# markosski/immutable3

Measured on AMD Instinct MI355X. Metric: scanned rows/sec + %HBM-roofline, 100M-row RangeFilter, 1/2/4/8 MI355X, higher is better.
Workload: dtype i32; 1 GPU; C2@100M: RangeFilter GT(2^28) AND LT(3*2^28) over one 100M-row DENSE_INT segment -> selection bitmap + selected-row count; block_rows=1024, segments_rotated_per_gpu=3, parallelism=1 GPU

## Files before the change

immutable3_amd/csrc/imm3_api.cpp:

```cpp
#include "../../include/imm3.h"
#include "../../include/imm3_diag.h"
#include "imm3_internal.h"
#include "../host/codec.hpp"

#include <algorithm>
#include <cmath>
#include <map>
#include <mutex>
#include <unordered_map>
#include <cstdio>
#include <cstring>
#include <functional>
#include <memory>
#include <string>
#include <vector>

#include "imm3_handles.h"
#include "imm3_distinct_plan.h"
#include "imm3_api_internal.h"

using namespace imm3;

static thread_local std::string g_err;

// ... 636 lines not shown
    const size_t bytes = (size_t)rows * 2 + kPad;
    void *p = nullptr, *pm = nullptr;
    if (rows < 1 || hipMalloc(&p, bytes) != hipSuccess || hipMalloc(&pm, 2 * sizeof(int32_t)) != hipSuccess) {
        (void)hipGetLastError();
        if (p) (void)hipFree(p);
        sc.hi16_state = -1;
        return IMM3_OK;
    }
    int32_t min_max[2] = {32767, -32768};
    hipError_t e = hipMemcpyAsync(pm, min_max, sizeof(min_max), hipMemcpyHostToDevice, ctx->stream);
    if (e == hipSuccess) e = hipMemsetAsync((uint8_t *)p + (size_t)rows * 2, 0, kPad, ctx->stream);
    if (e == hipSuccess) {
        LaunchTimer t(ctx, 5);
        launch_hi16_build((const int32_t *)sc.d_data, (int16_t *)p, rows, (int32_t *)pm, ctx->stream, t.start, t.stop);
        e = hipGetLastError();
    }
    if (e == hipSuccess) e = hipMemcpyAsync(min_max, pm, sizeof(min_max), hipMemcpyDeviceToHost, ctx->stream);
    if (e == hipSuccess) e = hipStreamSynchronize(ctx->stream);
    (void)hipFree(pm);
    if (e != hipSuccess) {
        (void)hipFree(p);
        HIPCHK(e);
    }
    if (!hi16_span_ok(min_max[0], min_max[1])) {
        (void)hipFree(p);
        sc.hi16_state = -1;
        return IMM3_OK;
    }
    sc.d_hi16 = (uint8_t *)p;
    sc.hi16_state = 1;
    seg->device_bytes += bytes;
    return IMM3_OK;
}

static int segment_await(imm3_ctx *ctx, const imm3_segment *seg) {
    if (seg->ready_pending.load(std::memory_order_acquire)) HIPCHK(hipStreamWaitEvent(ctx->stream, seg->ready, 0));
    return IMM3_OK;
}

static int segment_build(imm3_ctx *ctx, const imm3_column *cols, int32_t ncols, bool wrap, imm3_segment **out, bool async = false) {
    if (!out) return fail(IMM3_ERR_ARG, "null argument");
    *out = nullptr;
    CTX_LIVE(ctx);
    if (ncols <= 0 || !cols) return fail(IMM3_ERR_ARG, "a segment needs at least one column");
    HIPCHK(hipSetDevice(ctx->device));
    std::unique_ptr<imm3_segment, void (*)(imm3_segment *)> seg(new imm3_segment(), segment_free);
// ... 70 lines not shown
    }
    for (void *p : seg->registered) unpin_range(seg->ctx, p);
    seg->registered.clear();
    return IMM3_OK;
}

extern "C" int imm3_segment_destroy(imm3_segment *seg) {
    if (!seg) return IMM3_OK;
    if (seg->closed) return fail(IMM3_ERR_STATE, "segment destroyed twice");
    imm3_ctx *ctx = seg->ctx;
    ctx_retain(ctx);
    struct Unref { imm3_ctx *c; ~Unref() { ctx_release(c); } } unref{ctx};
    imm3::GateScope gate(&ctx->gate);
    if (!ctx->closed && ctx->capture) return fail(IMM3_ERR_STATE, "a graph capture is open on this context");
    seg->closed = true;
    if (!seg->ctx->closed) {
        (void)hipSetDevice(seg->ctx->device);
        if (seg->ready_pending.load()) (void)hipEventSynchronize(seg->ready);
        (void)hipStreamSynchronize(seg->ctx->stream);
    }
    for (void *p : seg->registered) unpin_range(seg->ctx, p);
    seg->registered.clear();
    segment_release(seg);
    return IMM3_OK;
}

extern "C" int imm3_segment_bytes(const imm3_segment *seg, uint64_t *device_bytes) {
    if (!seg || !device_bytes) return fail(IMM3_ERR_ARG, "null argument");
    *device_bytes = seg->device_bytes;
    return IMM3_OK;
}

static void table_release(const imm3_table *t);

static void query_free(imm3_query *q) {
    if (!q) return;
    imm3_ctx *ctx = q->ctx;
    if (!ctx) { delete q; return; }
    (void)hipSetDevice(ctx->device);
    if (ctx->aux && q->total_on_aux) (void)hipStreamSynchronize(ctx->aux);
    pool_release(ctx, q->d_bitmap);
    pool_release(ctx, q->d_tile_offsets);
    pool_release(ctx, q->d_chunk_sums);
    pool_release(ctx, q->d_block_partials);
    pool_release(ctx, q->d_limit_state);
    pool_release(ctx, q->d_total);
// ... 1072 lines not shown
            const size_t j = (size_t)(which - IMM3_PTR_ORDER_COLUMN);
            *ptr = j < q->d_order_proj.size() ? q->d_order_proj[j] : nullptr;
            return IMM3_OK;
        }
        if (which >= 16 && (size_t)(which - 16) < q->d_proj.size()) {
            *ptr = q->d_proj[(size_t)(which - 16)];
            return IMM3_OK;
        }
        return fail(IMM3_ERR_ARG, "unknown device pointer id");
    }
}

extern "C" int imm3_query_plan(const imm3_query *q, int64_t *out, int32_t n) {
    if (!q || !out) return fail(IMM3_ERR_ARG, "null argument");
    const int64_t v[15] = {q->single_pass ? 1 : 0, q->sp_P, q->sp_grid, q->sp_spans, q->d_stage_rec ? 1 : 0,
                           (q->single_pass || q->d_stage_rec) ? rec_layout(q->stage_kinds, -1).dwords : 0, q->run.ran_single_pass ? 1 : 0, (int64_t)q->run_syncs,
                           (int64_t)q->sp_abandoned_runs, (int64_t)q->sp_busy_runs, (int64_t)q->limit_gather_gave_up,
                           (int64_t)q->order_select_runs, (int64_t)q->order_full_runs, (int64_t)q->order_launches,
                           q->hi16_ran ? 1 : 0};
    for (int32_t i = 0; i < n && i < 15; ++i) out[i] = v[i];
    return IMM3_OK;
}

static int query_create_agg_impl(imm3_ctx *ctx, const imm3_segment *seg, const imm3_table *table,
                                 const int32_t *used_cols, int32_t n_used,
                                 const imm3_select *sels, int32_t n_sels,
                                 const int32_t *group_cols, int32_t n_group,
                                 const imm3_aggregate *aggs, int32_t n_aggs,
                                 int32_t table_block_size, imm3_query **out, bool wide_keys,
                                 const int32_t *prog = nullptr, int32_t n_prog = 0, bool tree = false) {
    if (!out) return fail(IMM3_ERR_ARG, "out is null");
    *out = nullptr;
    if (n_group < 0 || n_group > kMaxGroupCols || (n_group > 0 && !group_cols)) return fail(IMM3_ERR_ARG, "0..4 group columns are supported on the GPU path");
    if (n_aggs < 1 || n_aggs > kMaxAggs || !aggs) return fail(IMM3_ERR_ARG, "1..4 aggregates are supported on the GPU path");
    imm3_query *q = nullptr;
    std::vector<int32_t> row_cols(group_cols, group_cols + n_group);
    for (int32_t j = 0; j < n_aggs; ++j) row_cols.push_back(aggs[j].column);
    int rc = query_create_impl(ctx, seg, table, used_cols, n_used, sels, n_sels, nullptr, 0, 0, table_block_size, row_cols, &q, prog, n_prog, tree);
    if (rc) return rc;
    std::unique_ptr<imm3_query, void (*)(imm3_query *)> guard(q, query_free);
    int key_bytes = 0;
    for (int32_t g = 0; g < n_group; ++g) {
        if (group_cols[g] < 0 || group_cols[g] >= n_used) return fail(IMM3_ERR_ARG, "group column is not among the used columns");
        key_bytes += seg->cols[(size_t)q->used[(size_t)group_cols[g]]].width;
    }
    if (!wide_keys && key_bytes > 8) return fail(IMM3_ERR_ARG, "group key wider than 8 bytes is not supported on the GPU path");
// ... 540 lines not shown
```

immutable3_amd/csrc/imm3_handles.h:

```cpp
#pragma once

#include "../../include/imm3.h"
#include "imm3_internal.h"
#include "imm3_plan.h"
#include "imm3_sync.h"

#include <atomic>
#include <map>
#include <memory>
#include <mutex>
#include <string>
#include <unordered_map>
#include <vector>

namespace imm3 {
int fail(int code, const std::string &msg);
}
using imm3::fail;

#define HIPCHK(expr)                                                                              \
    do {                                                                                          \
        hipError_t _e = (expr);                                                                   \
        if (_e != hipSuccess)                                                                     \
            return fail(IMM3_ERR_DEVICE, std::string(#expr) + ": " + hipGetErrorString(_e));      \
// ... 112 lines not shown
static inline int32_t value_codec(int32_t c) {
    if (c == IMM3_PFOR_INT || c == IMM3_SNAPPY_INT) return IMM3_DENSE_INT;
    if (c == IMM3_SNAPPY_TINYINT) return IMM3_DENSE_TINYINT;
    if (c == IMM3_SNAPPY_STRING) return IMM3_DENSE_STRING;
    return c;
}

struct SegCol {
    int32_t codec = 0, width = 0;
    int32_t vcodec = 0;
    uint8_t *d_data = nullptr;
    bool owned = false;
    uint64_t bytes = 0;
    std::vector<int32_t> offsets;
    std::vector<int32_t> block_rows;
    int32_t in_cap = 0, out_cap = 0;
    int64_t rows = 0;
    bool tile_aligned = false;
    uint32_t *d_block_off = nullptr;
    uint32_t *d_row_base = nullptr;
    uint8_t *d_dense = nullptr;
    uint8_t *d_hi16 = nullptr;
    int32_t hi16_state = 0;
};

struct SegLayout {
    std::vector<int32_t> size;
    std::vector<int64_t> word_off;
    int64_t rows = 0, words = 0;
    bool ragged = false;
};

struct imm3_segment {
    std::atomic<int> refs{1};
    std::atomic<bool> closed{false};
    imm3_ctx *ctx = nullptr;
    std::vector<SegCol> cols;
    uint64_t device_bytes = 0;
    std::vector<void *> registered;
    hipEvent_t ready = nullptr;
    std::atomic<bool> ready_pending{false};
    std::mutex decode_mu;
    std::mutex layout_mu;
    std::map<int32_t, std::shared_ptr<const SegLayout>> layouts;
    std::map<std::pair<int32_t, int32_t>, bool> same_blocks;
    std::map<int32_t, void **> d_sample_ptrs;
// ... 185 lines not shown
```

immutable3_amd/csrc/imm3_internal.h:

```cpp
#pragma once

#include <hip/hip_runtime.h>
#include <stdint.h>
#include <algorithm>

#include "imm3_int_list_plan.h"
#include "imm3_hi16_plan.h"

#ifdef IMM3_ABLATE
#define IMM3_ABLATED(args, value) ((args).ablate == (value))
#define IMM3_ABLATE_BIT(args, bit) (((args).ablate & (bit)) != 0)
#else
#define IMM3_ABLATED(args, value) false
#define IMM3_ABLATE_BIT(args, bit) false
#endif

namespace imm3 {

constexpr int kTileRows = 1024;
constexpr int kTileWords = 16;
constexpr int kWavesPerBlock = 4;
constexpr int kBlockThreads = 256;
constexpr int kChunkTiles = 256;
constexpr int kSpanTiles = 16;
// ... 19 lines not shown
    int32_t list;
    int32_t list_empty;
    uint32_t list_mask, list_shift, list_max_probe;
};

enum TileKind : int32_t { TK_I32 = 0, TK_I8 = 1, TK_S2 = 2, TK_NONE = 3, TK_H16 = 4 };
constexpr int tile_kind_rank(int kind) { return kind == TK_H16 ? 3 : (kind == TK_NONE ? 4 : kind); }
constexpr int kMaxTileCols = 3;
constexpr int kDeferLines = 64;
constexpr int kMaxTileMatch = 8;
constexpr int kMaxArenaSlots = 256;

struct TileCol {
    const void *data;
    int32_t lo, hi;
    int32_t n_match;
    int32_t negated;
    uint32_t match[kMaxTileMatch];
};
IMM3_HOST_DEVICE inline const void *tile_col_full(const TileCol &c) { return (const void *)(uintptr_t)(((uint64_t)c.match[5] << 32) | (uint64_t)c.match[4]); }
inline void tile_col_set_full(TileCol &c, const void *full) {
    c.match[4] = (uint32_t)(uintptr_t)full;
    c.match[5] = (uint32_t)((uint64_t)(uintptr_t)full >> 32);
}

struct TileArgs {
    TileCol cols[kMaxTileCols];
    int32_t kinds[kMaxTileCols];
    int32_t and_existing;
    int32_t defer_lines;
    int32_t ablate;
    int64_t n_rows, n_words, n_tiles;
    uint64_t *bitmap;
    uint32_t *block_partials;
    unsigned long long *finish;
    void *stage_rec;
    uint32_t *tile_start;
    int64_t wave_cap;
    int32_t max_slots;
    int32_t chunked;
    unsigned long long *stamps;
    const uint32_t *tile_rows;
    const void *const *tile_ptrs[kMaxTileCols];
};

struct RecField {
// ... 89 lines not shown
};
void launch_emit(const EmitArgs &a, int n_gather, int grid_blocks, hipStream_t s, hipEvent_t ev0, hipEvent_t ev1);

constexpr int kProjectMinP = 1;
constexpr int kProjectMaxP = 64;
#ifndef IMM3_PROJECT_STREAMERS
#define IMM3_PROJECT_STREAMERS 8
#endif
#ifndef IMM3_PROJECT_RING_KB
#define IMM3_PROJECT_RING_KB 14
#endif
constexpr int kProjectStreamers = IMM3_PROJECT_STREAMERS;
constexpr int kProjectWriters = 4;
constexpr int kProjectRingBytes = IMM3_PROJECT_RING_KB * 1024;
constexpr int kFinishStatus = 2;
constexpr unsigned long long kStatusPfor = 1ULL, kStatusAbandoned = 2ULL, kStatusBusy = 4ULL;
constexpr int kStatusEpochShift = 8;
constexpr unsigned long long kStatusEpochMask = 0xFFFFFFULL;
constexpr int kFinishEpoch = 8;
constexpr int kFinishDense = 9;
constexpr int kFinishLimitRows = 11;
constexpr int kFinishLimitTiles = 12;
constexpr int kFinishLimitGaveUp = 13;
constexpr int kFinishLimitTicketLineWord = 8;
constexpr int kTableLimitMaxGrid = 512;
constexpr int kTableLimitClaimTiles = 32;
static_assert(kTableLimitClaimTiles % kSpanTiles == 0 && kTableLimitClaimTiles % kWavesPerBlock == 0, "the scanned prefix ends on a span boundary; a claim splits evenly over the waves");
constexpr int kDescValueBits = 36, kDescFlagShift = 36, kDescEpochShift = 38;
constexpr unsigned long long kDescValueMask = (1ULL << kDescValueBits) - 1;
constexpr unsigned long long kDescEpochMask = (1ULL << (64 - kDescEpochShift)) - 1;
constexpr uint32_t kProjectMaxPolls = 1u << 17;
struct ProjectTile {
    const void *p[kMaxTileCols];
    uint32_t rows;
    uint32_t pad;
};
struct ProjectArgs {
    TileCol cols[kMaxTileCols];
    int32_t kinds[kMaxTileCols];
    int32_t P;
    int64_t n_rows, n_tiles, n_spans;
    int64_t n_rounds;
    uint64_t *bitmap;
    unsigned long long *finish;
    unsigned long long *desc;
    unsigned long long *round_total;
// ... 304 lines not shown
    uint32_t slots, mask;
    const unsigned long long *recs;
    uint32_t n_recs;
    unsigned long long *out_recs;
    unsigned long long *out_n;
    uint32_t out_cap;
};
void launch_mergew_pack(const MergeWideArgs &a, hipStream_t s);
void launch_mergew_init(const MergeWideArgs &a, hipStream_t s);
void launch_mergew_insert(const MergeWideArgs &a, hipStream_t s);
void launch_mergew_collect(const MergeWideArgs &a, hipStream_t s);
void launch_group_collect(const AggArgs &a, hipStream_t s);
void launch_strmax_init(const AggArgs &a, hipStream_t s);
void launch_strmax_refine(const AggArgs &a, int j, int k, hipStream_t s, hipEvent_t ev0, hipEvent_t ev1);
void launch_strmax_collect(const AggArgs &a, int j, uint32_t n_groups, uint8_t *out, hipStream_t s);
void launch_distinct_mark(const AggArgs &a, int j, hipStream_t s, hipEvent_t ev0, hipEvent_t ev1);
void launch_group_keys(const AggArgs &a, uint32_t n_groups, int key_bytes, uint8_t *out, hipStream_t s);

constexpr int kSubTallies = 32;
constexpr int kFinishWords = 16 + kSubTallies * 16;
constexpr int kFinishLimitTicket = 16 + 16 * (kSubTallies - 1) + kFinishLimitTicketLineWord;
static_assert(kFinishLimitTicket < kFinishWords && kFinishLimitTicketLineWord > 0 && kFinishLimitTicketLineWord < 16, "the ticket word lies inside the finish block, beside the last sub-tally");
constexpr int kMaxFilterGrid = 4096;
int filter_grid(int64_t units, bool generic, bool any_i32, int grid_blocks, int narrow_row_bytes = 0);
struct PforArgs {
    const uint8_t *data;
    const uint32_t *block_off;
    const uint32_t *row_base;
    int64_t n_blocks;
    int32_t lo, hi;
    int32_t and_existing;
    int32_t pad;
    int64_t n_rows, n_words, n_tiles;
    uint64_t *bitmap;
    uint32_t *block_partials;
    int32_t *out;
    uint32_t *status;
};
void launch_hi16_build(const int32_t *src, int16_t *dst, int64_t n_rows, int32_t *min_max, hipStream_t s, hipEvent_t ev0, hipEvent_t ev1);
void launch_pfor_counts(const uint8_t *data, const uint32_t *block_off, int64_t n_blocks, int32_t *counts, hipStream_t s);
void launch_filter_pfor(const PforArgs &a, int grid, hipStream_t s, hipEvent_t ev0, hipEvent_t ev1);
void launch_pfor_decode(const PforArgs &a, int grid, hipStream_t s, hipEvent_t ev0, hipEvent_t ev1);

struct SnappyArgs {
    const uint8_t *data;
    const uint32_t *block_off;
    const uint32_t *row_base;
// ... 213 lines not shown
```

immutable3_amd/csrc/imm3_kernels.hip:

```cpp
#include "imm3_internal.h"
#include "imm3_device.h"
#include "imm3_tile.h"
#include <hip/hip_ext.h>

namespace imm3 {

struct Arena {
    uint32_t buf_n = 0;
    uint32_t arena_n = 0;
    uint32_t slot = 0;
    uint32_t last = 0;
};
constexpr int kArenaBufBytes = 8 * 1024;
constexpr int arena_buf_bytes(int R) { return R == 1 ? 4 * 1024 : kArenaBufBytes; }
constexpr int kArenaSlots = kMaxArenaSlots;

template <int R>
__device__ __forceinline__ void arena_flush(const TileArgs &a, Arena &A, const uint8_t *lds, int64_t wave_id, int lane) {
    typedef typename RecVec<R>::type vec;
    if (!A.buf_n) return;
    const vec *l = (const vec *)lds;
    vec *out = (vec *)a.stage_rec + wave_id * a.wave_cap + A.arena_n;
    lds_wave_order();
    if (!IMM3_ABLATED(a, 20))
// ... 89 lines not shown
    else c.load(data, row0, lane);
}

template <int K0, int K1, int K2, bool STAGE>
__device__ __forceinline__ uint32_t finish_full_tile(const TileArgs &a, int64_t tile, int lane, ColRegs<K0> &c0,
                                                     ColRegs<K1> &c1, ColRegs<K2> &c2, uint8_t *xp, uint8_t *lds, uint32_t *tstart, Arena &A,
                                                     int64_t wave_id, uint64_t *park = nullptr, const uint64_t *earlier = nullptr) {
    if constexpr (lane_tile(K0, K1, K2, STAGE) == 2) {
        const uint32_t m = c0.lane_mask(a.cols[0]) & c1.lane_mask(a.cols[1]) & c2.lane_mask(a.cols[2]);
        constexpr int kH16 = K0 == TK_H16 ? 0 : (K1 == TK_H16 ? 1 : (K2 == TK_H16 ? 2 : -1));
        bool refine = false;
        uint32_t und = 0;
        if constexpr (kH16 >= 0) {
            und = m & (lane_undecided(c0) | lane_undecided(c1) | lane_undecided(c2));
            refine = ballot64(und != 0u) != 0ULL;
        }
        if (!a.bitmap && !refine) return (uint32_t)__popc(m);
        uint32_t lo_a, lo_b, hi_a, hi_b;
        lane_runs_to_halves(m, lo_a, lo_b, hi_a, hi_b);
        const bool owner = (lane & 7) == 0;
        const int64_t wl = tile * kTileWords + (lane >> 3);
        uint64_t word_a = ((uint64_t)hi_a << 32) | (uint64_t)lo_a, word_b = ((uint64_t)hi_b << 32) | (uint64_t)lo_b;
        if constexpr (kH16 >= 0) {
            if (refine) refine_undecided(a.cols[kH16], tile * kTileRows, lane, und, word_a, word_b);
            if (!a.bitmap) return owner ? (uint32_t)(__popcll(word_a) + __popcll(word_b)) : 0u;
        }
        if (a.and_existing) {
            word_a &= owner ? a.bitmap[wl] : 0ULL;
            word_b &= owner ? a.bitmap[wl + kTileWords / 2] : 0ULL;
        }
        if (!owner) word_a = word_b = 0;
        if (owner) {
            if (park) {
                park[lane >> 3] = word_a;
                park[kTileWords / 2 + (lane >> 3)] = word_b;
            } else {
                __builtin_nontemporal_store(word_a, a.bitmap + wl);
                __builtin_nontemporal_store(word_b, a.bitmap + wl + kTileWords / 2);
            }
        }
        return (uint32_t)(__popcll(word_a) + __popcll(word_b));
    } else if constexpr (lane_tile(K0, K1, K2, STAGE) == 1) {
        const uint32_t m = c0.lane_mask(a.cols[0]) & c1.lane_mask(a.cols[1]) & c2.lane_mask(a.cols[2]);
        if (!a.bitmap) return (uint32_t)__popc(m);
        const uint32_t odd = (uint32_t)__builtin_amdgcn_mov_dpp((int)m, 0xF5, 0xF, 0xF, true);
        const uint32_t pair = m | (odd << 16);
        const uint32_t high = (uint32_t)__builtin_amdgcn_mov_dpp((int)pair, 0xAA, 0xF, 0xF, true);
// ... 186 lines not shown
    for (int64_t grp = wave_id; grp < n_groups; grp += n_waves) {
        ColRegs<K0> c0[T];
        ColRegs<K1> c1[T];
        ColRegs<K2> c2[T];
        uint64_t earlier[T];
        if constexpr (kPipe) {
#pragma unroll
            for (int t = 0; t < T; ++t) {
                c0[t] = n0[t];
                c1[t] = n1[t];
                c2[t] = n2[t];
                c0[t].touch();
                c1[t].touch();
                c2[t].touch();
            }
            if constexpr (!STAGE) {
#pragma unroll
                for (int t = 0; t < T; ++t) {
                    if constexpr (kLane == 2) earlier[t] = ~0ULL;
                    else if constexpr (kLane == 1) earlier[t] = a.and_existing ? a.bitmap[(grp * T + t) * kTileWords + (lane >> 2)] : ~0ULL;
                    else earlier[t] = (a.and_existing && lane < kTileWords) ? a.bitmap[(grp * T + t) * kTileWords + lane] : (a.and_existing ? 0ULL : ~0ULL);
                }
            }
            load_group(n0, n1, n2, grp + n_waves < n_groups ? grp + n_waves : grp);
            if constexpr (STAGE)
                if (arena_full<kRecDwords>(A, 2 * A.last)) arena_flush<kRecDwords>(a, A, lds, wave_id, lane);
        } else {
            load_group(c0, c1, c2, grp);
        }
        if (DEFER && parked == 0) first_grp = grp;
#pragma unroll
        for (int t = 0; t < T; ++t)
            lane_total += finish_full_tile<K0, K1, K2, STAGE>(a, grp * T + t, lane, c0[t], c1[t], c2[t], xp, lds, tstart, A, wave_id, DEFER ? park + (parked + t) * kTileWords : nullptr,
                                                              (kPipe && !STAGE && kLane != 2) ? &earlier[t] : nullptr);
        if (DEFER) {
            parked += T;
            if (parked + T > a.defer_lines) flush();
        }
    }
    if (DEFER && parked) flush();
    for (int64_t tile = n_groups * T + wave_id; tile < n_tiles_here; tile += n_waves) {
        const int64_t row0 = tile * kTileRows;
        ColRegs<K0> c0;
        ColRegs<K1> c1;
        ColRegs<K2> c2;
        if (tile < n_full) {
            tile_load<kLane>(c0, a.cols[0].data, row0, lane);
// ... 541 lines not shown
    const int lane = threadIdx.x & 63;
    const int wave = threadIdx.x >> 6;
    int32_t acc = 0;
    for (int64_t tile = (int64_t)blockIdx.x * kWavesPerBlock + wave; tile < n_tiles; tile += (int64_t)gridDim.x * kWavesPerBlock) {
        const int32_t *p = data + tile * kTileRows + lane;
        int32_t v[kTileWords];
#pragma unroll
        for (int j = 0; j < kTileWords; ++j) v[j] = __builtin_nontemporal_load(p + 64 * j);
#pragma unroll
        for (int j = 0; j < kTileWords; ++j) acc ^= v[j];
    }
    if (acc == 0x5A5A5A5A) *sink = acc;
}

void launch_read_stream(const int32_t *data, int64_t n_tiles, int32_t *sink, hipStream_t s, hipEvent_t ev0, hipEvent_t ev1) {
    IMM3_LAUNCH(k_read_stream, 512, kBlockThreads, s, ev0, ev1, data, n_tiles, sink);
}

static inline int clamp_grid(int64_t want, int cap) {
    if (want < 1) want = 1;
    return (int)(want > cap ? cap : want);
}

int filter_grid(int64_t units, bool generic, bool any_i32, int grid_blocks, int narrow_row_bytes) {
    const int narrow = narrow_row_bytes <= 1 ? 1536 : (narrow_row_bytes == 2 ? 768 : 512);
    const int dflt = generic ? 2048 : (any_i32 ? 512 : narrow);
    const int cap = grid_blocks > 0 ? (grid_blocks > kMaxFilterGrid ? kMaxFilterGrid : grid_blocks) : dflt;
    return clamp_grid((units + kWavesPerBlock - 1) / kWavesPerBlock, cap);
}


#define IMM3_TILE_CASE(k0, k1, k2, T)                                                           \
    if (a.kinds[0] == k0 && a.kinds[1] == k1 && a.kinds[2] == k2) {                             \
        if (!a.bitmap && a.defer_lines) return false;  \
        else if (a.stage_rec && a.tile_rows) return false;             \
        else if (a.stage_rec && a.defer_lines) IMM3_LAUNCH_LDS((k_filter_tile<k0, k1, k2, T, false, true, true>), grid, kBlockThreads, \
                             (size_t)kWavesPerBlock * (size_t)a.defer_lines * kTileWords * sizeof(uint64_t), s, ev0, ev1, a); \
        else if (a.stage_rec) IMM3_LAUNCH((k_filter_tile<k0, k1, k2, T, false, false, true>), grid, kBlockThreads, s, ev0, ev1, a); \
        else if (a.tile_rows && a.defer_lines) IMM3_LAUNCH_LDS((k_filter_tile<k0, k1, k2, 1, true, true, false>), grid, kBlockThreads, \
                             (size_t)kWavesPerBlock * (size_t)a.defer_lines * (kTileWords + 1) * sizeof(uint64_t), s, ev0, ev1, a); \
        else if (a.tile_rows) IMM3_LAUNCH((k_filter_tile<k0, k1, k2, 1, true, false, false>), grid, kBlockThreads, s, ev0, ev1, a); \
        else if (a.defer_lines) IMM3_LAUNCH_LDS((k_filter_tile<k0, k1, k2, T, false, true, false>), grid, kBlockThreads,       \
                             (size_t)kWavesPerBlock * (size_t)a.defer_lines * kTileWords * sizeof(uint64_t), s, ev0, ev1, a); \
        else IMM3_LAUNCH((k_filter_tile<k0, k1, k2, T, false, false, false>), grid, kBlockThreads, s, ev0, ev1, a); \
        return true;                                                                            \
    }

#define IMM3_TILE_CASE_H16(k0, k1, k2, T)                                                       \
// ... 13 lines not shown
    X(TK_I32, TK_I32, TK_I32, 1) X(TK_I32, TK_I32, TK_I8, 1) X(TK_I32, TK_I8, TK_I8, 1)              \
    X(TK_I8, TK_I8, TK_I8, 2) X(TK_I32, TK_I32, TK_S2, 1) X(TK_I32, TK_I8, TK_S2, 1) X(TK_I8, TK_I8, TK_S2, 1)

#define IMM3_TILE_KINDS_H16(X) X(TK_H16, TK_NONE, TK_NONE, 1) X(TK_I8, TK_H16, TK_NONE, 1)

bool launch_filter_tile(const TileArgs &a, int grid, hipStream_t s, hipEvent_t ev0, hipEvent_t ev1) {
    IMM3_TILE_KINDS(IMM3_TILE_CASE)
    IMM3_TILE_KINDS_H16(IMM3_TILE_CASE_H16)
    return false;
}

bool launch_filter_table_limit(const TileArgs &a, int grid, hipStream_t s, hipEvent_t ev0, hipEvent_t ev1) {
    if (!a.tile_rows || !a.bitmap || !a.finish || a.and_existing || a.stage_rec) return false;
#define IMM3_TABLE_LIMIT_CASE(k0, k1, k2, T)                                                    \
    if (a.kinds[0] == k0 && a.kinds[1] == k1 && a.kinds[2] == k2) {                             \
        IMM3_LAUNCH((k_filter_table_limit<k0, k1, k2>), grid, kBlockThreads, s, ev0, ev1, a);   \
        return true;                                                                            \
    }
    IMM3_TILE_KINDS(IMM3_TABLE_LIMIT_CASE)
#undef IMM3_TABLE_LIMIT_CASE
    return false;
}

__global__ __launch_bounds__(kBlockThreads) void k_hi16_build(const int32_t *src, int16_t *dst, int64_t n_rows, int32_t *min_max) {
    const int64_t n8 = n_rows / 8;
    int32_t mn = 32767, mx = -32768;
    const IMM3_GLOBAL v4i *in = (const IMM3_GLOBAL v4i *)src;
    IMM3_GLOBAL v4i *out = (IMM3_GLOBAL v4i *)dst;
    for (int64_t i = (int64_t)blockIdx.x * kBlockThreads + threadIdx.x; i < n8; i += (int64_t)gridDim.x * kBlockThreads) {
        const v4i x = __builtin_nontemporal_load(in + 2 * i), y = __builtin_nontemporal_load(in + 2 * i + 1);
        const int32_t h[8] = {x[0] >> 16, x[1] >> 16, x[2] >> 16, x[3] >> 16, y[0] >> 16, y[1] >> 16, y[2] >> 16, y[3] >> 16};
        v4i o;
#pragma unroll
        for (int k = 0; k < 4; ++k) {
            o[k] = (int32_t)(((uint32_t)h[2 * k] & 0xFFFFu) | ((uint32_t)h[2 * k + 1] << 16));
            mn = min(mn, min(h[2 * k], h[2 * k + 1]));
            mx = max(mx, max(h[2 * k], h[2 * k + 1]));
        }
        out[i] = o;
    }
    const int64_t tail = 8 * n8 + threadIdx.x;
    if (blockIdx.x == 0 && threadIdx.x < 8 && tail < n_rows) {
        const int32_t h = src[tail] >> 16;
        dst[tail] = (int16_t)h;
        mn = min(mn, h);
        mx = max(mx, h);
    }
#pragma unroll
    for (int d = 32; d >= 1; d >>= 1) {
        mn = min(mn, __shfl_xor(mn, d));
        mx = max(mx, __shfl_xor(mx, d));
    }
    if ((threadIdx.x & 63) == 0) {
        atomicMin(min_max, mn);
        atomicMax(min_max + 1, mx);
    }
}

void launch_hi16_build(const int32_t *src, int16_t *dst, int64_t n_rows, int32_t *min_max, hipStream_t s, hipEvent_t ev0, hipEvent_t ev1) {
    const int grid = clamp_grid((n_rows / 8 + kBlockThreads - 1) / kBlockThreads, 2048);
    IMM3_LAUNCH(k_hi16_build, grid, kBlockThreads, s, ev0, ev1, src, dst, n_rows, min_max);
}

int filter_tile_group(const int32_t *kinds) {
#define IMM3_TILE_T(k0, k1, k2, T) \
    if (kinds[0] == k0 && kinds[1] == k1 && kinds[2] == k2) return T;
    IMM3_TILE_KINDS(IMM3_TILE_T)
    IMM3_TILE_KINDS_H16(IMM3_TILE_T)
#undef IMM3_TILE_T
    return 0;
}

void launch_filter_generic(const FilterArgs &a, int grid, hipStream_t s, hipEvent_t ev0, hipEvent_t ev1) {
    IMM3_LAUNCH(k_filter_generic, grid, kBlockThreads, s, ev0, ev1, a);
}

void launch_total(const TotalArgs &a, hipStream_t s, hipEvent_t ev0, hipEvent_t ev1) {
    IMM3_LAUNCH(k_total, 1, 64, s, ev0, ev1, a);
}

__global__ __launch_bounds__(kChunkTiles) void k_limit_gather(const LimitGatherArgs a) {
    __shared__ uint32_t s_wave[kChunkTiles / 64];
    __shared__ uint32_t s_chunk_total[kLimitGatherMaxChunks];
// ... 169 lines not shown
```

immutable3_amd/csrc/imm3_run.cpp:

```cpp
#include "../../include/imm3.h"
#include "../../include/imm3_diag.h"
#include "imm3_internal.h"

#include <algorithm>
#include <cstring>
#include <mutex>
#include <vector>

#include "imm3_handles.h"
#include "imm3_api_internal.h"

using namespace imm3;

void imm3::fill_colpred(const imm3_query *q, const FoldedPred &fp, ColPred &cp) {
    std::memset(&cp, 0, sizeof(cp));
    const SegCol &sc = q->seg->cols[(size_t)fp.seg_col];
    cp.data = col_flat(sc);
    cp.kind = fp.kind;
    cp.width = fp.width;
    cp.lo = (int32_t)fp.lo;
    cp.hi = (int32_t)fp.hi;
    cp.n_match = (int32_t)fp.match.size();
    cp.negated = fp.negated ? 1 : 0;
    cp.match_in_args = (fp.kind == KIND_STR && !fp.d_blob) ? 1 : 0;
// ... 43 lines not shown
    bool chunked = false;
    int pass = 0;
    int grid = 1;
    bool count_done = false;
};

template <class Args> static void fill_bitmap_tail(const imm3_query *q, Args &a) {
    a.n_rows = q->n_rows;
    a.n_words = q->n_words;
    a.n_tiles = q->n_tiles;
    a.bitmap = q->d_bitmap;
    a.block_partials = q->d_block_partials;
}
template <class Args> static void fill_pass_tail(const imm3_query *q, const SelectRun &run, Args &a) {
    a.and_existing = run.pass > 0;
    fill_bitmap_tail(q, a);
}

static int tile_kind_bytes(int kind) { return kind == TK_I32 ? 4 : ((kind == TK_S2 || kind == TK_H16) ? 2 : (kind == TK_I8 ? 1 : 0)); }

struct TileGridHint {
    bool any_i32 = false;
    int narrow_bytes = 0;
};
static TileGridHint tile_grid_hint(const int32_t *kinds) {
    TileGridHint h;
    for (int k = 0; k < kMaxTileCols; ++k) {
        h.any_i32 |= kinds[k] == TK_I32;
        if (kinds[k] != TK_I32) h.narrow_bytes += tile_kind_bytes(kinds[k]);
    }
    return h;
}

static unsigned long long *claim_stamp_slot(imm3_ctx *ctx, int grid) {
    if (!ctx->d_stamps) return nullptr;
    std::lock_guard<std::mutex> lk(ctx->mu);
    if (!ctx->d_stamps || ctx->stamp_used >= ctx->stamp_slots) return nullptr;
    unsigned long long *slot = ctx->d_stamps + (size_t)ctx->stamp_used * kMaxFilterGrid * 2;
    ctx->stamp_grids.push_back(grid);
    ++ctx->stamp_used;
    return slot;
}

static LimitScanInputs limit_scan_inputs(const imm3_query *q, const SelectRun &run) {
    LimitScanInputs li;
    li.whole = run.mode & SEL_WHOLE;
    li.count_log_on = q->count_log_on;
    li.count_in_scan = run.count_in_scan;
    li.limit = q->limit;
    li.single_tile_pass = run.chain.single_tile_pass;
    li.table = q->table != nullptr;
    li.records = q->d_stage_rec != nullptr;
    li.skip_bitmap = run.skip_bitmap;
// ... 93 lines not shown
        in.n_s2 += tk == TK_S2;
    }
    return in;
}

static void take_hi16_plane(imm3_query *q, const SelectRun &run, const std::vector<const FoldedPred *> &take, TileArgs &a) {
    for (int k = 0; k < (int)take.size() && k < kMaxTileCols; ++k) {
        if (a.kinds[k] != TK_I32) continue;
        const FoldedPred &fp = *take[(size_t)k];
        if (!fp.d_hi16) return;
        Hi16Inputs in = hi16_inputs(q, fp, take);
        in.stages = a.stage_rec != nullptr;
        in.chunked = run.chunked || (q->limit > 0 && run.count_in_scan && !(run.mode & SEL_WHOLE));
        in.pinned_i32 = run.fv == TV_I32_SCAN;
        if (!hi16_eligible(in)) return;
        TileCol &c = a.cols[k];
        tile_col_set_full(c, c.data);
        c.data = fp.d_hi16;
        const Hi16Bounds b = hi16_bounds(c.lo, c.hi);
        c.match[0] = b.possible_first;
        c.match[1] = b.possible_count;
        c.match[2] = b.certain_first;
        c.match[3] = b.certain_count;
        a.kinds[k] = TK_H16;
        for (int j = k; j + 1 < kMaxTileCols && tile_kind_rank(a.kinds[j + 1]) < tile_kind_rank(a.kinds[j]); ++j) {
            std::swap(a.kinds[j], a.kinds[j + 1]);
            std::swap(a.cols[j], a.cols[j + 1]);
        }
        q->hi16_ran = true;
        return;
    }
}

static int fill_tile_args(imm3_query *q, SelectRun &run, const std::vector<const FoldedPred *> &take, TileArgs &a) {
    imm3_ctx *ctx = q->ctx;
    std::memset(&a, 0, sizeof(a));
    const int n = (int)take.size();
    for (int k = 0; k < kMaxTileCols; ++k) a.kinds[k] = TK_NONE;
    for (int k = 0; k < n; ++k) {
        const FoldedPred &fp = *take[(size_t)k];
        if (q->table) a.tile_ptrs[k] = (const void *const *)q->table->d_tile_ptrs[(size_t)fp.seg_col];
        a.kinds[k] = tile_kind(fp);
        fill_tile_col(q, fp, a.cols[k], a.kinds[k]);
    }
    if (run.chain.single_tile_pass && q->d_stage_rec && !run.skip_bitmap && !(run.mode & SEL_PLAIN)) {
        bool same = true;
        for (int k = 0; k < kMaxTileCols; ++k) same = same && a.kinds[k] == q->stage_kinds[k] && (k >= n || take[(size_t)k]->seg_col == q->stage_seg_col[k]);
        if (!same) return fail(IMM3_ERR_ARG, "internal: staged record layout does not match the tile launch");
        a.stage_rec = q->d_stage_rec;
        a.tile_start = q->d_tile_start;
        a.wave_cap = q->stage_wave_cap;
        a.max_slots = q->stage_max_slots;
        q->run.stage_written = true;
    }
    take_hi16_plane(q, run, take, a);
    a.ablate = tile_ablation(run.fv);
    fill_pass_tail(q, run, a);
    q->run.bitmap_lazy = q->run.stage_written && run.count_in_scan && !q->count_log_on && run.fv != TV_EAGER_BITMAP;
    if (q->run.bitmap_lazy) {
        a.bitmap = nullptr;
        q->run.bitmap_valid = false;
    }
    a.tile_rows = q->table ? q->table->d_tile_rows : nullptr;
    const TileGridHint hint = tile_grid_hint(a.kinds);
    run.grid = filter_grid(q->n_tiles, false, hint.any_i32, ctx->grid_blocks, hint.narrow_bytes);
    if (q->run.stage_written) run.grid = q->stage_grid;
    if (run.chain.single_tile_pass && !run.overlap_total && run.fv != TV_COUNT_BY_K_TOTAL && (run.grid <= 512 || run.fv != TV_COUNT_SMALL_GRID)) {
        a.finish = q->d_total;
        run.count_done = true;
    }
    a.defer_lines = (run.fv == TV_PLAN_PINNED || q->run.bitmap_lazy) ? 0 : (q->run.stage_written ? 16 : (run.grid <= 1024 ? kDeferLines : 16));
    if (run.skip_bitmap) {
        a.bitmap = nullptr;
        a.defer_lines = 0;
    }
    return IMM3_OK;
}

static int launch_tile_table_limit(imm3_query *q, SelectRun &run, TileArgs &a, int grid) {
    imm3_ctx *ctx = q->ctx;
    run.grid = grid;
    a.stamps = claim_stamp_slot(ctx, run.grid);
    a.finish = q->d_total;
    a.defer_lines = 0;
    LaunchTimer t(ctx, 0);
    if (!launch_filter_table_limit(a, run.grid, run.s, t.start, t.stop)) return fail(IMM3_ERR_ARG, "internal: no tile kernel for this column combination");
    HIPCHK(hipGetLastError());
    run.count_done = true;
// ... 842 lines not shown
```

immutable3_amd/native.py:

```python
from __future__ import annotations

import ctypes as C
import os
import threading
import weakref
from typing import List, Optional, Sequence

import numpy as np

_PKG = os.path.dirname(os.path.abspath(__file__))
LIB_PATH = os.path.join(_PKG, "lib", "libimm3.so")

PFOR_INT, DENSE_INT, DENSE_TINYINT, DENSE_STRING = 0, 1, 2, 3
SNAPPY_INT, SNAPPY_TINYINT, SNAPPY_STRING = 16, 17, 18
INT_CODECS, TINYINT_CODECS = (DENSE_INT, PFOR_INT, SNAPPY_INT), (DENSE_TINYINT, SNAPPY_TINYINT)
MATCH, NOTMATCH, EQ, GT, LT, NOOP = 0, 1, 2, 3, 4, 5
STR_RANGE = 6
INT_IN = 7
INT_IN_MAX_VALUES = 1 << 24
INT_LIST_I8, INT_LIST_ARGS, INT_LIST_LDS, INT_LIST_GLOBAL = 0, 1, 2, 3
EXPR_AND, EXPR_OR, EXPR_NOT = -1, -2, -4
EXPR_FORM_TILE, EXPR_FORM_GENERIC = 0, 1
TABLE_TREE_REFUSED = "a select tree over a table takes "
MERGE_VIEW_REFUSED = "a view of merged groups takes "
# ... 10 lines not shown
    "imm3_query_segment_starts", "imm3_query_locate_rows",
    "imm3_query_create", "imm3_query_create_agg", "imm3_query_group_count", "imm3_query_fetch_groups", "imm3_query_agg_shape",
    "imm3_query_fetch_group_strings", "imm3_query_destroy", "imm3_query_reserve_rows", "imm3_query_set_order", "imm3_query_set_group_order",
    "imm3_query_set_group_filter",
    "imm3_query_create_agg_wide", "imm3_query_create_table_agg_wide", "imm3_query_fetch_group_keys",
    "imm3_query_create_expr", "imm3_query_create_agg_expr", "imm3_query_create_table_expr", "imm3_query_create_table_agg_expr",
    "imm3_query_run", "imm3_query_run_select", "imm3_query_run_count", "imm3_query_sync", "imm3_query_join_count", "imm3_query_log_counts",
    "imm3_query_layout", "imm3_query_batches", "imm3_query_count", "imm3_query_bitmap",
    "imm3_query_row_count", "imm3_query_fetch_rows", "imm3_query_device_ptr",
    "imm3_comm_unique_id", "imm3_comm_create", "imm3_comm_create_all", "imm3_comm_destroy", "imm3_comm_info",
    "imm3_comm_sync", "imm3_comm_join", "imm3_comm_allreduce_u64", "imm3_comm_allreduce_count", "imm3_comm_allreduce_count_all", "imm3_comm_merge_groups", "imm3_comm_merge_groups_all",
    "imm3_comm_merge_groups_wide", "imm3_comm_merge_groups_wide_all", "imm3_comm_merge_ordered", "imm3_comm_merge_ordered_all",
    "imm3_comm_merge_groups_view", "imm3_comm_merge_groups_view_all",
    "imm3_pfor_encode_bound", "imm3_pfor_encode_block", "imm3_pfor_encode_column",
    "imm3_snappy_encode_bound", "imm3_snappy_encode_block",
]
DIAG_EXPORTS = [
    "imm3_ctx_timing_enable", "imm3_ctx_timing_reset", "imm3_ctx_timing_mask", "imm3_ctx_timing_collect", "imm3_ctx_set_tuning",
    "imm3_ctx_measure_read_gbps", "imm3_ctx_devclock_enable", "imm3_ctx_devclock_collect", "imm3_ctx_devclock_raw", "imm3_query_plan",
    "imm3_ctx_inject_fault", "imm3_ctx_debug_device_lock", "imm3_plan_predict", "imm3_comm_debug_standin", "imm3_plan_limit_scan",
    "imm3_plan_table_limit", "imm3_plan_string_route", "imm3_plan_string_range_route", "imm3_plan_limit_chunks", "imm3_plan_distinct_capacity",
    "imm3_plan_int_list_table", "imm3_plan_int_list_form", "imm3_plan_int_list_probe",
    "imm3_plan_hi16_bounds", "imm3_plan_hi16_class", "imm3_plan_hi16_span_ok", "imm3_plan_hi16_eligible",
    "imm3_query_agg_form", "imm3_query_expr_form", "imm3_expr_normalize", "imm3_query_group_order_path",
    "imm3_query_group_filter_stats", "imm3_group_filter_check", "imm3_comm_merge_view_path", "imm3_merge_view_plan_json",
]
COMM_ID_BYTES = 128
PTR_ORDER_ROW_INDEX, PTR_ORDER_ROW_COUNT, PTR_ORDER_COLUMN = 0x1000, 0x1001, 0x2000
GROUP_ORDER_GROUP_COL, GROUP_ORDER_AGG = 0, 1
GROUP_ORDER_KEY_MAX_WIDTH = 12
ORDER_MAX_KEYS = 4
GROUP_ORDER_NONE, GROUP_ORDER_SMALL, GROUP_ORDER_RADIX_FULL, GROUP_ORDER_RADIX_SELECT = 0, 1, 2, 3
GROUP_ORDER_SMALL_MAX = 2048
GROUP_FILTER_COUNT = -1
GROUP_FILTER_MAX_LEAVES, GROUP_FILTER_MAX_PROG = 8, 32
GROUP_FILTER_LEAF = np.dtype([("agg", "<i4"), ("average", "<i4"), ("cond", "<i4"), ("value", "<i8")], align=True)
TV_I32_SCAN = 26
TV_GROUP_ORDER_RADIX = 25
TV_ORDER_FULL_SORT, TV_ORDER_SELECT_ALWAYS = 23, 24


def group_filter_arrays(leaves: Sequence[tuple], prog: Sequence[int]):
    ls = np.zeros(max(len(leaves), 1), GROUP_FILTER_LEAF)
    for i, (agg, average, cond, value) in enumerate(leaves):
        ls[i] = (int(agg), 1 if average else 0, int(cond), int(value))
    pg = np.array(list(prog) or [0], dtype=np.int32)
    return ls, pg
# ... 409 lines not shown
    return arr, keep


class DeviceSegment:

    def __init__(self, ctx: Context, cols, wrap_device: bool = False, async_copy: bool = False):
        self.ctx = ctx
        self.ncols = len(cols)
        arr, keep = _ccolumns(cols)
        self._h = C.c_void_p()
        fn = load().imm3_segment_wrap_device if wrap_device else (load().imm3_segment_create_async if async_copy else load().imm3_segment_create)
        _check(fn(ctx._h, arr, len(cols), C.byref(self._h)))
        ctx._adopt(self)
        self._keep = keep if (wrap_device or async_copy) else None
        self.widths = [c[1] for c in cols]
        self.codecs = [c[0] for c in cols]

    @property
    def device_bytes(self) -> int:
        n = C.c_uint64(0)
        _check(load().imm3_segment_bytes(self._h, C.byref(n)))
        return n.value

    def wait(self):
        _check(load().imm3_segment_wait(self._h))

    def close(self):
        if self._h:
            load().imm3_segment_destroy(self._h)
            self._h = C.c_void_p()

    def __del__(self):
        try:
            self.close()
        except Exception:
            pass


AGG_COUNT, AGG_MIN, AGG_MAX, AGG_SUM = 0, 1, 2, 3
AGG_COUNT_DISTINCT = 5
KERNEL_DISTINCT_MARK, KERNEL_DISTINCT_CLEAR = 10, 11
AGG_FORM_LANES, AGG_FORM_LANES_WIDE, AGG_FORM_DIRECT, AGG_FORM_TILE, AGG_FORM_GENERAL = 0, 1, 2, 3, 4
GROUP_KEY_MAX_WIDTH = 256
TV_AGG_WEAK_HASH = 18
TV_NO_LIMIT_CHUNKS = 14
TABLE_LIMIT_CLAIM_TILES = 32
# ... 346 lines not shown
        out = np.zeros((max(g, 1), width), np.uint8)
        _check(load().imm3_query_fetch_group_strings(self._h, j, out.ctypes.data, g))
        return out[:g]

    def fetch_group_keys(self) -> np.ndarray:
        n = C.c_uint32(0)
        _check(load().imm3_query_group_count(self._h, C.byref(n)))
        g = n.value
        kb = C.c_int32(0)
        _check(load().imm3_query_agg_shape(self._h, None, None, C.byref(kb)))
        out = np.zeros((max(g, 1), max(kb.value, 1)), np.uint8)
        _check(load().imm3_query_fetch_group_keys(self._h, out.ctypes.data, g))
        return out[:g, : kb.value]

    def plan(self) -> dict:
        v = np.zeros(15, np.int64)
        _check(load().imm3_query_plan(self._h, v.ctypes.data, 15))
        return {"single_pass": bool(v[0]), "P": int(v[1]), "grid": int(v[2]), "spans": int(v[3]), "records": bool(v[4]),
                "rec_dwords": int(v[5]), "ran_single_pass": bool(v[6]), "run_syncs": int(v[7]),
                "abandoned_runs": int(v[8]), "busy_runs": int(v[9]), "limit_gather_gave_up": int(v[10]),
                "order_select_runs": int(v[11]), "order_full_runs": int(v[12]), "order_launches": int(v[13]),
                "hi16_plane": bool(v[14])}

    def agg_form(self) -> int:
        f = C.c_int32(-1)
        _check(load().imm3_query_agg_form(self._h, C.byref(f)))
        return f.value

    def expr_form(self) -> int:
        f = C.c_int32(-1)
        _check(load().imm3_query_expr_form(self._h, C.byref(f)))
        return f.value

    def device_ptr(self, which: int) -> int:
        p = C.c_void_p()
        _check(load().imm3_query_device_ptr(self._h, which, C.byref(p)))
        return p.value or 0

    def close(self):
        if self._h:
            load().imm3_query_destroy(self._h)
            self._h = C.c_void_p()

    def __del__(self):
        try:
            self.close()
# ... 266 lines not shown
```

include/imm3_diag.h:

```cpp
#ifndef IMM3_DIAG_H
#define IMM3_DIAG_H

#include "imm3.h"

#ifdef __cplusplus
extern "C" {
#endif

int imm3_ctx_timing_enable(imm3_ctx *ctx, int32_t max_records);
int imm3_ctx_timing_reset(imm3_ctx *ctx);
int imm3_ctx_timing_mask(imm3_ctx *ctx, uint32_t kernel_mask);
int imm3_ctx_timing_collect(imm3_ctx *ctx, int32_t kernel_id, float *ms_out, int32_t cap, int32_t *n_out);

int imm3_ctx_devclock_enable(imm3_ctx *ctx, int32_t max_launches);
int imm3_ctx_devclock_collect(imm3_ctx *ctx, float *ms_out, int32_t cap, int32_t *n_out);
int imm3_ctx_devclock_raw(imm3_ctx *ctx, int32_t launch, uint64_t *out, int32_t n);

int imm3_ctx_measure_read_gbps(imm3_ctx *ctx, uint64_t bytes, int32_t iters, double *gbps);

int imm3_ctx_set_tuning(imm3_ctx *ctx, int32_t filter_variant, int32_t grid_blocks);

int imm3_plan_predict(int64_t n_rows, const int32_t *pred_width, const int32_t *pred_match, int32_t n_pred, const int32_t *proj_width,
                      const int32_t *proj_is_pred, int32_t n_proj, int32_t rec_bytes, double sigma, double sloc, double full, double *out_abc);

int imm3_query_plan(const imm3_query *q, int64_t *out, int32_t n);

int imm3_query_agg_form(const imm3_query *q, int32_t *form);

#define IMM3_GROUP_ORDER_SMALL_MAX 2048
int imm3_query_group_order_path(const imm3_query *q, int32_t *path);

int imm3_comm_merge_view_path(const imm3_comm *c, int32_t *path);

int imm3_merge_view_plan_json(int32_t n_group, const int32_t *group_kind, const int32_t *group_width, int32_t n_aggs, const int32_t *agg_kind,
                              const int32_t *agg_col_kind, const int32_t *agg_col_width, const imm3_group_view *view, uint32_t largest_segment_index,
                              char *json_out, int64_t cap, int64_t *needed);

int imm3_query_group_filter_stats(const imm3_query *q, uint64_t *groups_in, uint64_t *groups_kept);

int imm3_group_filter_check(int32_t is_agg, const int32_t *agg_kind, const int32_t *agg_col_kind, int32_t n_aggs, const imm3_group_filter_leaf *leaves,
                            int32_t n_leaves, const int32_t *prog, int32_t n_prog, const int64_t *count_vals, int32_t *kept);

int imm3_query_expr_form(const imm3_query *q, int32_t *form);

int imm3_expr_normalize(const int32_t *col_codec, const int32_t *col_width, int32_t n_cols, const imm3_select *leaves, int32_t n_leaves,
                        const int32_t *prog, int32_t n_prog, char *json_out, int64_t cap, int64_t *needed);

int imm3_plan_limit_scan(int32_t whole, int32_t count_log_on, int32_t count_in_scan, int64_t limit, int32_t single_tile_pass, int32_t table, int32_t records,
// ... 24 lines not shown
```

Measured before the change: 2451 billion rows/s.

## Tune hi16 plane scan grid, unroll hi16 build, add refine diagnostics

Gives the filter a dedicated grid cap when the hi16 plane is the only tile column. The tail prefetch in the grouped loop now reloads group 0 instead of repeating the current group when the plane is scanned. The hi16 build kernel is unrolled four times with nontemporal stores and launches a smaller grid. It also adds diagnostics: a device flag recording whether the undecided-row refinement ran, plus an API that reads back the hi16 plane and its min/max. The flag store adds one global write per refined tile.

```diff
diff --git a/immutable3_amd/csrc/imm3_api.cpp b/immutable3_amd/csrc/imm3_api.cpp
--- a/immutable3_amd/csrc/imm3_api.cpp
+++ b/immutable3_amd/csrc/imm3_api.cpp
@@ -682,6 +682,8 @@
         (void)hipFree(p);
         HIPCHK(e);
     }
+    sc.hi16_min = min_max[0];
+    sc.hi16_max = min_max[1];
     if (!hi16_span_ok(min_max[0], min_max[1])) {
         (void)hipFree(p);
         sc.hi16_state = -1;
@@ -798,6 +800,19 @@
     for (void *p : seg->registered) unpin_range(seg->ctx, p);
     seg->registered.clear();
     segment_release(seg);
+    return IMM3_OK;
+}
+
+extern "C" int imm3_segment_hi16_plane(const imm3_segment *seg, int32_t col, int16_t *out, int64_t cap_rows, int32_t *state, int32_t *min_max) {
+    if (!seg || !state || !min_max || col < 0 || (size_t)col >= seg->cols.size()) return fail(IMM3_ERR_ARG, "bad argument");
+    const SegCol &sc = seg->cols[(size_t)col];
+    *state = sc.hi16_state;
+    min_max[0] = sc.hi16_min;
+    min_max[1] = sc.hi16_max;
+    if (sc.hi16_state == 1 && out) {
+        const int64_t rows = (int64_t)(sc.bytes / 4);
+        HIPCHK(hipMemcpy(out, sc.d_hi16, (size_t)(rows < cap_rows ? rows : cap_rows) * sizeof(int16_t), hipMemcpyDeviceToHost));
+    }
     return IMM3_OK;
 }
 
@@ -1916,6 +1931,19 @@
     return IMM3_OK;
 }
 
+extern "C" int imm3_query_hi16_refined(imm3_query *q, int32_t *refined) {
+    if (!q || !refined) return fail(IMM3_ERR_ARG, "null argument");
+    if (q->ctx->capture) return fail(IMM3_ERR_STATE, "a graph capture is open");
+    *refined = 0;
+    if (!q->d_total) return IMM3_OK;
+    unsigned long long w = 0;
+    HIPCHK(hipMemcpyAsync(&w, q->d_total + kFinishHi16Refined, sizeof(w), hipMemcpyDeviceToHost, q->ctx->stream));
+    HIPCHK(hipStreamSynchronize(q->ctx->stream));
+    if (w) HIPCHK(hipMemsetAsync(q->d_total + kFinishHi16Refined, 0, sizeof(w), q->ctx->stream));
+    *refined = w ? 1 : 0;
+    return IMM3_OK;
+}
+
 static int query_create_agg_impl(imm3_ctx *ctx, const imm3_segment *seg, const imm3_table *table,
                                  const int32_t *used_cols, int32_t n_used,
                                  const imm3_select *sels, int32_t n_sels,
diff --git a/immutable3_amd/csrc/imm3_handles.h b/immutable3_amd/csrc/imm3_handles.h
--- a/immutable3_amd/csrc/imm3_handles.h
+++ b/immutable3_amd/csrc/imm3_handles.h
@@ -158,6 +158,7 @@
     uint8_t *d_dense = nullptr;
     uint8_t *d_hi16 = nullptr;
     int32_t hi16_state = 0;
+    int32_t hi16_min = 32767, hi16_max = -32768;
 };
 
 struct SegLayout {
diff --git a/immutable3_amd/csrc/imm3_internal.h b/immutable3_amd/csrc/imm3_internal.h
--- a/immutable3_amd/csrc/imm3_internal.h
+++ b/immutable3_amd/csrc/imm3_internal.h
@@ -65,6 +65,11 @@
 inline void tile_col_set_full(TileCol &c, const void *full) {
     c.match[4] = (uint32_t)(uintptr_t)full;
     c.match[5] = (uint32_t)((uint64_t)(uintptr_t)full >> 32);
+}
+IMM3_HOST_DEVICE inline unsigned long long *tile_col_refined(const TileCol &c) { return (unsigned long long *)(uintptr_t)(((uint64_t)c.match[7] << 32) | (uint64_t)c.match[6]); }
+inline void tile_col_set_refined(TileCol &c, unsigned long long *word) {
+    c.match[6] = (uint32_t)(uintptr_t)word;
+    c.match[7] = (uint32_t)((uint64_t)(uintptr_t)word >> 32);
 }
 
 struct TileArgs {
@@ -200,6 +205,7 @@
 constexpr int kFinishLimitRows = 11;
 constexpr int kFinishLimitTiles = 12;
 constexpr int kFinishLimitGaveUp = 13;
+constexpr int kFinishHi16Refined = 14;
 constexpr int kFinishLimitTicketLineWord = 8;
 constexpr int kTableLimitMaxGrid = 512;
 constexpr int kTableLimitClaimTiles = 32;
@@ -550,7 +556,7 @@
 constexpr int kFinishLimitTicket = 16 + 16 * (kSubTallies - 1) + kFinishLimitTicketLineWord;
 static_assert(kFinishLimitTicket < kFinishWords && kFinishLimitTicketLineWord > 0 && kFinishLimitTicketLineWord < 16, "the ticket word lies inside the finish block, beside the last sub-tally");
 constexpr int kMaxFilterGrid = 4096;
-int filter_grid(int64_t units, bool generic, bool any_i32, int grid_blocks, int narrow_row_bytes = 0);
+int filter_grid(int64_t units, bool generic, bool any_i32, int grid_blocks, int narrow_row_bytes = 0, bool lone_plane = false);
 struct PforArgs {
     const uint8_t *data;
     const uint32_t *block_off;
diff --git a/immutable3_amd/csrc/imm3_kernels.hip b/immutable3_amd/csrc/imm3_kernels.hip
--- a/immutable3_amd/csrc/imm3_kernels.hip
+++ b/immutable3_amd/csrc/imm3_kernels.hip
@@ -135,7 +135,10 @@
         const int64_t wl = tile * kTileWords + (lane >> 3);
         uint64_t word_a = ((uint64_t)hi_a << 32) | (uint64_t)lo_a, word_b = ((uint64_t)hi_b << 32) | (uint64_t)lo_b;
         if constexpr (kH16 >= 0) {
-            if (refine) refine_undecided(a.cols[kH16], tile * kTileRows, lane, und, word_a, word_b);
+            if (refine) {
+                if (lane == 0) *tile_col_refined(a.cols[kH16]) = 1ULL;
+                refine_undecided(a.cols[kH16], tile * kTileRows, lane, und, word_a, word_b);
+            }
             if (!a.bitmap) return owner ? (uint32_t)(__popcll(word_a) + __popcll(word_b)) : 0u;
         }
         if (a.and_existing) {
@@ -368,7 +371,8 @@
                     else earlier[t] = (a.and_existing && lane < kTileWords) ? a.bitmap[(grp * T + t) * kTileWords + lane] : (a.and_existing ? 0ULL : ~0ULL);
                 }
             }
-            load_group(n0, n1, n2, grp + n_waves < n_groups ? grp + n_waves : grp);
+            constexpr bool kPlane = K0 == TK_H16 || K1 == TK_H16 || K2 == TK_H16;
+            load_group(n0, n1, n2, grp + n_waves < n_groups ? grp + n_waves : (kPlane ? (int64_t)0 : grp));
             if constexpr (STAGE)
                 if (arena_full<kRecDwords>(A, 2 * A.last)) arena_flush<kRecDwords>(a, A, lds, wave_id, lane);
         } else {
@@ -956,8 +960,9 @@
     return (int)(want > cap ? cap : want);
 }
 
-int filter_grid(int64_t units, bool generic, bool any_i32, int grid_blocks, int narrow_row_bytes) {
-    const int narrow = narrow_row_bytes <= 1 ? 1536 : (narrow_row_bytes == 2 ? 768 : 512);
+int filter_grid(int64_t units, bool generic, bool any_i32, int grid_blocks, int narrow_row_bytes, bool lone_plane) {
+    constexpr int kPlaneGrid = 1536;
+    const int narrow = lone_plane ? kPlaneGrid : (narrow_row_bytes <= 1 ? 1536 : (narrow_row_bytes == 2 ? 768 : 512));
     const int dflt = generic ? 2048 : (any_i32 ? 512 : narrow);
     const int cap = grid_blocks > 0 ? (grid_blocks > kMaxFilterGrid ? kMaxFilterGrid : grid_blocks) : dflt;
     return clamp_grid((units + kWavesPerBlock - 1) / kWavesPerBlock, cap);
@@ -1017,22 +1022,39 @@
     return false;
 }
 
+__device__ __forceinline__ v4i hi16_pack8(const v4i x, const v4i y, int32_t &mn, int32_t &mx) {
+    const int32_t h[8] = {x[0] >> 16, x[1] >> 16, x[2] >> 16, x[3] >> 16, y[0] >> 16, y[1] >> 16, y[2] >> 16, y[3] >> 16};
+    v4i o;
+#pragma unroll
+    for (int k = 0; k < 4; ++k) {
+        o[k] = (int32_t)(((uint32_t)h[2 * k] & 0xFFFFu) | ((uint32_t)h[2 * k + 1] << 16));
+        mn = min(mn, min(h[2 * k], h[2 * k + 1]));
+        mx = max(mx, max(h[2 * k], h[2 * k + 1]));
+    }
+    return o;
+}
+
 __global__ __launch_bounds__(kBlockThreads) void k_hi16_build(const int32_t *src, int16_t *dst, int64_t n_rows, int32_t *min_max) {
+    constexpr int kUnroll = 4;
     const int64_t n8 = n_rows / 8;
     int32_t mn = 32767, mx = -32768;
     const IMM3_GLOBAL v4i *in = (const IMM3_GLOBAL v4i *)src;
     IMM3_GLOBAL v4i *out = (IMM3_GLOBAL v4i *)dst;
-    for (int64_t i = (int64_t)blockIdx.x * kBlockThreads + threadIdx.x; i < n8; i += (int64_t)gridDim.x * kBlockThreads) {
+    const int64_t stride = (int64_t)gridDim.x * kBlockThreads;
+    int64_t i = (int64_t)blockIdx.x * kBlockThreads + threadIdx.x;
+    for (; i + (kUnroll - 1) * stride < n8; i += kUnroll * stride) {
+        v4i x[kUnroll], y[kUnroll];
+#pragma unroll
+        for (int u = 0; u < kUnroll; ++u) {
+            x[u] = __builtin_nontemporal_load(in + 2 * (i + u * stride));
+            y[u] = __builtin_nontemporal_load(in + 2 * (i + u * stride) + 1);
+        }
+#pragma unroll
+        for (int u = 0; u < kUnroll; ++u) __builtin_nontemporal_store(hi16_pack8(x[u], y[u], mn, mx), out + (i + u * stride));
+    }
+    for (; i < n8; i += stride) {
         const v4i x = __builtin_nontemporal_load(in + 2 * i), y = __builtin_nontemporal_load(in + 2 * i + 1);
-        const int32_t h[8] = {x[0] >> 16, x[1] >> 16, x[2] >> 16, x[3] >> 16, y[0] >> 16, y[1] >> 16, y[2] >> 16, y[3] >> 16};
-        v4i o;
-#pragma unroll
-        for (int k = 0; k < 4; ++k) {
-            o[k] = (int32_t)(((uint32_t)h[2 * k] & 0xFFFFu) | ((uint32_t)h[2 * k + 1] << 16));
-            mn = min(mn, min(h[2 * k], h[2 * k + 1]));
-            mx = max(mx, max(h[2 * k], h[2 * k + 1]));
-        }
-        out[i] = o;
+        __builtin_nontemporal_store(hi16_pack8(x, y, mn, mx), out + i);
     }
     const int64_t tail = 8 * n8 + threadIdx.x;
     if (blockIdx.x == 0 && threadIdx.x < 8 && tail < n_rows) {
@@ -1053,7 +1075,8 @@
 }
 
 void launch_hi16_build(const int32_t *src, int16_t *dst, int64_t n_rows, int32_t *min_max, hipStream_t s, hipEvent_t ev0, hipEvent_t ev1) {
-    const int grid = clamp_grid((n_rows / 8 + kBlockThreads - 1) / kBlockThreads, 2048);
+    const int64_t per_group = (int64_t)kBlockThreads * 4;
+    const int grid = clamp_grid((n_rows / 8 + per_group - 1) / per_group, 2048);
     IMM3_LAUNCH(k_hi16_build, grid, kBlockThreads, s, ev0, ev1, src, dst, n_rows, min_max);
 }
 
diff --git a/immutable3_amd/csrc/imm3_run.cpp b/immutable3_amd/csrc/imm3_run.cpp
--- a/immutable3_amd/csrc/imm3_run.cpp
+++ b/immutable3_amd/csrc/imm3_run.cpp
@@ -89,6 +89,7 @@
 struct TileGridHint {
     bool any_i32 = false;
     int narrow_bytes = 0;
+    bool lone_plane = false;
 };
 static TileGridHint tile_grid_hint(const int32_t *kinds) {
     TileGridHint h;
@@ -96,6 +97,7 @@
         h.any_i32 |= kinds[k] == TK_I32;
         if (kinds[k] != TK_I32) h.narrow_bytes += tile_kind_bytes(kinds[k]);
     }
+    h.lone_plane = kinds[0] == TK_H16 && kinds[1] == TK_NONE;
     return h;
 }
 
@@ -235,6 +237,7 @@
         c.match[1] = b.possible_count;
         c.match[2] = b.certain_first;
         c.match[3] = b.certain_count;
+        tile_col_set_refined(c, q->d_total + kFinishHi16Refined);
         a.kinds[k] = TK_H16;
         for (int j = k; j + 1 < kMaxTileCols && tile_kind_rank(a.kinds[j + 1]) < tile_kind_rank(a.kinds[j]); ++j) {
             std::swap(a.kinds[j], a.kinds[j + 1]);
@@ -276,7 +279,7 @@
     }
     a.tile_rows = q->table ? q->table->d_tile_rows : nullptr;
     const TileGridHint hint = tile_grid_hint(a.kinds);
-    run.grid = filter_grid(q->n_tiles, false, hint.any_i32, ctx->grid_blocks, hint.narrow_bytes);
+    run.grid = filter_grid(q->n_tiles, false, hint.any_i32, ctx->grid_blocks, hint.narrow_bytes, hint.lone_plane);
     if (q->run.stage_written) run.grid = q->stage_grid;
     if (run.chain.single_tile_pass && !run.overlap_total && run.fv != TV_COUNT_BY_K_TOTAL && (run.grid <= 512 || run.fv != TV_COUNT_SMALL_GRID)) {
         a.finish = q->d_total;
diff --git a/immutable3_amd/native.py b/immutable3_amd/native.py
--- a/immutable3_amd/native.py
+++ b/immutable3_amd/native.py
@@ -56,7 +56,7 @@
     "imm3_plan_table_limit", "imm3_plan_string_route", "imm3_plan_string_range_route", "imm3_plan_limit_chunks", "imm3_plan_distinct_capacity",
     "imm3_plan_int_list_table", "imm3_plan_int_list_form", "imm3_plan_int_list_probe",
     "imm3_plan_hi16_bounds", "imm3_plan_hi16_class", "imm3_plan_hi16_span_ok", "imm3_plan_hi16_eligible",
-    "imm3_query_agg_form", "imm3_query_expr_form", "imm3_expr_normalize", "imm3_query_group_order_path",
+    "imm3_query_agg_form", "imm3_query_hi16_refined", "imm3_segment_hi16_plane", "imm3_query_expr_form", "imm3_expr_normalize", "imm3_query_group_order_path",
     "imm3_query_group_filter_stats", "imm3_group_filter_check", "imm3_comm_merge_view_path", "imm3_merge_view_plan_json",
 ]
 COMM_ID_BYTES = 128
@@ -512,6 +512,15 @@
         _check(load().imm3_segment_bytes(self._h, C.byref(n)))
         return n.value
 
+    def hi16_plane(self, col: int, rows: int):
+        L = load()
+        L.imm3_segment_hi16_plane.argtypes = [C.c_void_p, C.c_int32, C.c_void_p, C.c_int64, C.POINTER(C.c_int32), C.c_void_p]
+        out = np.zeros(max(rows, 1), np.int16)
+        state = C.c_int32(0)
+        mm = np.zeros(2, np.int32)
+        _check(L.imm3_segment_hi16_plane(self._h, col, out.ctypes.data, rows, C.byref(state), mm.ctypes.data))
+        return state.value, (int(mm[0]), int(mm[1])), (out[:rows] if state.value == 1 else None)
+
     def wait(self):
         _check(load().imm3_segment_wait(self._h))
 
@@ -904,6 +913,13 @@
                 "order_select_runs": int(v[11]), "order_full_runs": int(v[12]), "order_launches": int(v[13]),
                 "hi16_plane": bool(v[14])}
 
+    def hi16_refined(self) -> bool:
+        L = load()
+        L.imm3_query_hi16_refined.argtypes = [C.c_void_p, C.POINTER(C.c_int32)]
+        r = C.c_int32(0)
+        _check(L.imm3_query_hi16_refined(self._h, C.byref(r)))
+        return bool(r.value)
+
     def agg_form(self) -> int:
         f = C.c_int32(-1)
         _check(load().imm3_query_agg_form(self._h, C.byref(f)))
diff --git a/include/imm3_diag.h b/include/imm3_diag.h
--- a/include/imm3_diag.h
+++ b/include/imm3_diag.h
@@ -24,6 +24,9 @@
                       const int32_t *proj_is_pred, int32_t n_proj, int32_t rec_bytes, double sigma, double sloc, double full, double *out_abc);
 
 int imm3_query_plan(const imm3_query *q, int64_t *out, int32_t n);
+
+int imm3_query_hi16_refined(imm3_query *q, int32_t *refined);
+int imm3_segment_hi16_plane(const imm3_segment *seg, int32_t col, int16_t *out, int64_t cap_rows, int32_t *state, int32_t *min_max);
 
 int imm3_query_agg_form(const imm3_query *q, int32_t *form);
 
```

After: 2543 billion rows/s (median of 6 runs). +3.7%, better.
